# Layjins/Spider

Measured on AMD Instinct MI355X. Metric: multimodal responses/sec (text->text+image), higher is better.
Workload: dtype bf16

## Files before the change

include/spider_hip.h:

```cpp
#ifndef SPIDER_HIP_H
#define SPIDER_HIP_H
#define SPIDER_ABI_VERSION 4

#ifdef __cplusplus
extern "C" {
#endif

int spider_abi_version(void);
const char* spider_target_arch(void);
const char* spider_last_error(void);


int spider_embed_bf16(const void* table, const int* ids, void* out, int rows, int H, int V, void* stream);

int spider_rmsnorm_bf16(const void* x, const void* res, const void* w, void* y, void* res_out, int rows, int H,
                        float eps, void* stream);

int spider_gemv_bf16(const void* W, const void* x, void* out, const void* bias, const void* res, const void* norm_w,
                     float eps, int B, int N, int K, void* stream);

int spider_gemv_swiglu_bf16(const void* W_gate_up, const void* x, void* out, const void* norm_w, float eps, int B,
                            int I, int K, void* stream);

int spider_lm_head_nparts(int V);
// ... 18 lines not shown
                                         const int* ngram, const void* ban, void* ban_step, int V, int cap, int B, void* stream);

int spider_beam_partial_bf16(const void* logits, float* ws_ms, float* ws_val, int* ws_tok, int rows, int V, int C, int nslice,
                             void* stream);
int spider_beam_select_f32(const float* ws_ms, const float* ws_val, const int* ws_tok, float* run_scores, const int* eos_ids,
                           const int* n_eos, const int* n_hist, float* trace_score, int* trace_beam, int* trace_tok, int cap,
                           int* src_beam, int* next_ids, int B, int K, int V, int C, int nslice, void* stream);
int spider_kv_row_gather_bf16(void* k_cache, void* v_cache, void* k_tmp, void* v_tmp, const int* src_beam, const int* kv_beg,
                              const int* kv_end, int K, int R, int layers, int rows_alloc, int n_kv, int T, int d, void* stream);

int spider_sample_partial_bf16(const void* logits, const void* seen, const void* ban, const float* penalty, const int* min_new,
                               const int* eos_ids, const int* n_eos, const int* n_hist, const int* top_k, float* ws_val,
                               int* ws_tok, int rows, int V, int nslice, void* stream);
int spider_sample_select_f32(const float* ws_val, const int* ws_tok, const float* temperature, const float* top_p, const int* top_k,
                             const void* seed, const int* row0, const int* n_hist, int* next_ids, int* cand_tok, float* cand_p,
                             int* n_keep, float* u, int rows, int V, int nslice, void* stream);

int spider_rope_kv_append_bf16(const void* qkv, const int* pos, const int* slot, const float* cos_sin, void* q_out,
                               void* k_cache, void* v_cache, int B, int S, int n_q, int n_kv, int d, int T_max,
                               void* stream);
int spider_rope_kv_append_mrope_bf16(const void* qkv, const int* pos3, const int* slot, const float* cos_sin, void* q_out,
                                     void* k_cache, void* v_cache, int B, int S, int n_q, int n_kv, int d, int T_max,
                                     int sec_t, int sec_h, void* stream);

int spider_attn_decode_bf16(const void* q, const void* k_cache, const void* v_cache, const int* kv_beg,
                            const int* kv_end, void* out, void* ws_o, void* ws_ml, int B, int n_q, int n_kv, int d,
                            int T_max, float scale, int nsplit, void* stream);

int spider_attn_decode_fused_bf16(const void* qkv, const int* pos, const float* cos_sin, void* k_cache, void* v_cache,
                                  const int* kv_beg, const int* kv_end, void* out, void* ws_o, void* ws_ml,
                                  int* counters, int B, int n_q, int n_kv, int d, int T_max, float scale, int nsplit,
                                  void* stream);
int spider_set_attn_inline(int on);
int spider_set_gemv_sched(int sched);
int spider_set_ws_inlaunch(int on);

int spider_gemv_fm_bf16(const void* Wfm, const void* x, void* out, const void* bias, const void* res, int B, int N, int K,
                        int fold_rmsnorm, float eps, void* stream);
int spider_gemv_swiglu_fm_bf16(const void* Wfm_gate_up, const void* x, void* out, int B, int I, int K, int fold_rmsnorm, float eps,
                               void* stream);
int spider_lm_head_argmax_fm_bf16(const void* Wfm, const void* x, int* out_ids, void* logits, void* ws_val, void* ws_idx, int B,
                                  int V, int K, int fold_rmsnorm, float eps, void* stream);
int spider_lm_head_argmax_fm_proc_bf16(const void* Wfm, const void* x, int* out_ids, void* logits, void* ws_val, void* ws_idx,
                                       const void* seen, const void* ban, const float* penalty, const int* min_new,
                                       const int* eos_ids, const int* n_eos, const int* n_hist, int B, int V, int K,
                                       int fold_rmsnorm, float eps, void* stream);


int spider_gemm_bf16(const void* A, const void* W, void* C, void* C32, const void* bias, const void* res,
                     const void* rowbias, int rows_per_group, int M, int N, int K, int lda, int ldc, int act,
                     float out_scale, int w_tiled, const float* res32, float* c32d, void* ws, long ws_bytes, void* stream);

int spider_gemm_ln_bf16(const void* A, const void* Wf, void* C, const float* colsum, const float* colbias, const void* res,
                        int M, int N, int K, int ldc, int act, float eps, int w_tiled, void* ws, long ws_bytes, void* stream);

int spider_xattn_fused_bf16(const void* x, const void* mq_fm, const void* mo_fm, const float* colsum, const float* colbias,
                            const void* bias_o, void* out, int B2, int n_tok, int C, int heads, int n_keys, float eps,
                            const float* x32, float* out32, void* stream);

int spider_conv2d_nhwc_bf16(const void* x, const void* w, void* y, const void* bias, const void* res,
                            const void* rowbias, int B, int Hin, int Win, int Cin, int Cout, int ks, int stride,
                            int pad, int ups, float out_scale, int w_tiled, const float* res32, float* c32d, void* ws, long ws_bytes, void* stream);

int spider_conv_nhwc_ex_bf16(const void* x, const void* w, void* y, const void* bias, const void* res,
                             const void* rowbias, int B, int Hin, int Win, int Cin, int Cout, int kh, int kw, int stride,
                             int pad_h, int pad_w, int dil, int up_h, int up_w, int act, float act_param,
// ... 183 lines not shown
```

spider_amd/csrc/common.hpp:

```cpp
#pragma once
#include <hip/hip_runtime.h>
#include <stdint.h>

namespace spider {

typedef uint16_t bf16_t;

typedef __attribute__((ext_vector_type(4))) float f32x4;
typedef __attribute__((ext_vector_type(16))) float f32x16;
typedef __attribute__((ext_vector_type(8))) short bf16x8;
typedef __attribute__((ext_vector_type(4))) short bf16x4;

typedef __attribute__((ext_vector_type(4))) uint32_t u32x4;
typedef __attribute__((ext_vector_type(2))) uint32_t u32x2;

__device__ __forceinline__ float bf16_to_f32(bf16_t v) {
    return __uint_as_float(((uint32_t)v) << 16);
}
__device__ __forceinline__ float bf16lo_to_f32(uint32_t packed) {
    return __uint_as_float(packed << 16);
}
__device__ __forceinline__ float bf16hi_to_f32(uint32_t packed) {
    return __uint_as_float(packed & 0xffff0000u);
}
// ... 48 lines not shown
__device__ __forceinline__ float h16hi_to_f32(uint32_t packed) { return bf16hi_to_f32(packed); }
__device__ __forceinline__ h16_t f32_to_h16(float f) { return f32_to_bf16(f); }
__device__ __forceinline__ uint32_t pack_h16x2(float lo, float hi) { return pack_bf16x2(lo, hi); }
__device__ __forceinline__ float dot2_h16(uint32_t a, uint32_t b, float acc) {
    return __builtin_amdgcn_fdot2_f32_bf16(__builtin_bit_cast(hw_bf16x2, a), __builtin_bit_cast(hw_bf16x2, b), acc, false);
}
__device__ __forceinline__ f32x4 mfma_16x16x32_h16(h16x8 a, h16x8 b, f32x4 c) {
    return __builtin_amdgcn_mfma_f32_16x16x32_bf16(a, b, c, 0, 0, 0);
}
__device__ __forceinline__ f32x16 mfma_32x32x16_h16(h16x8 a, h16x8 b, f32x16 c) {
    return __builtin_amdgcn_mfma_f32_32x32x16_bf16(a, b, c, 0, 0, 0);
}
__device__ __forceinline__ f32x4 mfma_16x16x16_h16(h16x4 a, h16x4 b, f32x4 c) {
    return __builtin_amdgcn_mfma_f32_16x16x16bf16_1k(a, b, c, 0, 0, 0);
}
#endif
#define SPIDER_FN(name) SPIDER_CAT2(name, SPIDER_DT)

__device__ __forceinline__ float dot2_bf16(uint32_t a, uint32_t b, float acc) {
    return __builtin_amdgcn_fdot2_f32_bf16(__builtin_bit_cast(hw_bf16x2, a), __builtin_bit_cast(hw_bf16x2, b), acc, false);
}

__device__ __forceinline__ float wave_sum(float v) {
#pragma unroll
    for (int o = 32; o > 0; o >>= 1) v += __shfl_xor(v, o, 64);
    return v;
}
__device__ __forceinline__ float wave_max(float v) {
#pragma unroll
    for (int o = 32; o > 0; o >>= 1) v = fmaxf(v, __shfl_xor(v, o, 64));
    return v;
}

template <int NW>
__device__ __forceinline__ float block_sum(float v, float* red) {
    v = wave_sum(v);
    const int lane = threadIdx.x & 63, w = threadIdx.x >> 6;
    __syncthreads();
    if (lane == 0) red[w] = v;
    __syncthreads();
    float t = 0.f;
#pragma unroll
    for (int i = 0; i < NW; ++i) t += red[i];
    return t;
}

__device__ __forceinline__ float silu_f(float x) { return x * __builtin_amdgcn_rcpf(1.f + __expf(-x)); }
__device__ __forceinline__ float erf_fast(float x) {
    const float ax = fabsf(x);
    const float t = __builtin_amdgcn_rcpf(fmaf(0.3275911f, ax, 1.f));
    float p = fmaf(1.061405429f, t, -1.453152027f);
    p = fmaf(p, t, 1.421413741f);
    p = fmaf(p, t, -0.284496736f);
    p = fmaf(p, t, 0.254829592f);
    const float e = 1.f - p * t * __expf(-ax * ax);
    return copysignf(e, x);
}
__device__ __forceinline__ float gelu_erf_f(float x) { return 0.5f * x * (1.f + erf_fast(x * 0.70710678118654752f)); }
__device__ __forceinline__ float quick_gelu_f(float x) { return x * __builtin_amdgcn_rcpf(1.f + __expf(-1.702f * x)); }

__device__ __forceinline__ int xcd_remap(int bid, int nwg) {
    const int q = nwg >> 3, r = nwg & 7, xcd = bid & 7, idx = bid >> 3;
    const int base = (xcd < r) ? xcd * (q + 1) : r * (q + 1) + (xcd - r) * q;
    return base + idx;
}

}

template <typename F>
// ... 28 lines not shown
```

spider_amd/csrc/llm_decode.hip:

```cpp
#include "common.hpp"
#include "select.hpp"
#include <stdlib.h>

using namespace spider;

__global__ __launch_bounds__(256) void embed_kernel(const bf16_t* __restrict__ table, const int* __restrict__ ids,
                                                    bf16_t* __restrict__ out, int H, int V) {
    const int r = blockIdx.x;
    int id = ids[r];
    id = id < 0 ? 0 : (id >= V ? V - 1 : id);
    const u32x4* src = reinterpret_cast<const u32x4*>(table + (size_t)id * H);
    u32x4* dst = reinterpret_cast<u32x4*>(out + (size_t)r * H);
    for (int i = threadIdx.x; i < H / 8; i += 256) dst[i] = src[i];
}

__global__ __launch_bounds__(256) void rope_rows_kernel(bf16_t* __restrict__ x, const float* __restrict__ cs, long row_stride,
                                                        int rows, int heads, int d) {
    const int half = d >> 1, cpr = half >> 3;
    const long total = (long)rows * heads * cpr;
    for (long idx = (long)blockIdx.x * 256 + threadIdx.x; idx < total; idx += (long)gridDim.x * 256) {
        const int c = (int)(idx % cpr);
        const int h = (int)((idx / cpr) % heads);
        const long r = idx / ((long)cpr * heads);
        bf16_t* p = x + r * row_stride + (long)h * d + c * 8;
// ... 218 lines not shown
                u32x4 ov;
                ov.x = o[0]; ov.y = o[1]; ov.z = o[2]; ov.w = o[3];
                sv[min(i0 + c * NT, nv - 1)] = ov;
            }
        };
        auto hoist_w = [&]() {
#pragma unroll
            for (int u = 0; u < H; ++u) {
                const int k = lane * 8 + u * 512;
#pragma unroll
                for (int r = 0; r < NR; ++r)
                    w0[u][r] = __builtin_nontemporal_load(reinterpret_cast<const u32x4*>(wrow[r] + (unsigned)(k < K ? k : K - 8)));
            }
        };
        const u32x4* xv = reinterpret_cast<const u32x4*>(x);
        u32x4* sv = reinterpret_cast<u32x4*>(xs);
        if (!XLDS) {
            hoist_w();
        } else if (!norm_w) {
            issue_x(xv, t0);
            hoist_w();
            store_x(sv, t0);
            asm volatile("" ::: "memory");
            for (int b = 0; b < NB; ++b)
                for (int i0 = b ? 0 : CAP * NT; i0 < nv; i0 += CAP * NT) {
                    issue_x(xv + (size_t)b * nv, i0 + t0);
                    store_x(sv + (size_t)b * nv, i0 + t0);
                }
        } else if (nv <= CH * NT) {
            issue_xw(xv, t0);
            hoist_w();
            for (int b = 0; b < NB; ++b) {
                if (b) issue_xw(xv + (size_t)b * nv, t0);
                const float rs = rsqrtf(block_sum<NWB>(sumsq(0.f, t0, CH), red) / (float)K + eps);
                norm_store(sv + (size_t)b * nv, t0, rs);
            }
        } else {
            hoist_w();
            for (int b = 0; b < NB; ++b) {
                float ss = 0.f;
                for (int i0 = 0; i0 < nv; i0 += CAP * NT) {
                    issue_x(xv + (size_t)b * nv, i0 + t0);
                    ss = sumsq(ss, i0 + t0, CAP);
                }
                const float rs = rsqrtf(block_sum<NWB>(ss, red) / (float)K + eps);
                for (int i0 = 0; i0 < nv; i0 += CH * NT) {
                    issue_xw(xv + (size_t)b * nv, i0 + t0);
                    norm_store(sv + (size_t)b * nv, i0 + t0, rs);
                }
            }
        }
        if (XLDS) __syncthreads();
    }

    if (col0 >= N) return;
    float acc[NB][NR];
#pragma unroll
    for (int b = 0; b < NB; ++b)
#pragma unroll
        for (int r = 0; r < NR; ++r) acc[b][r] = 0.f;

    auto fma_w = [&](const u32x4 (&wq)[U][NR], int k0) {
#pragma unroll
        for (int u = 0; u < U; ++u) {
            const int k = k0 + u * 512;
            if (k < K) {
#pragma unroll
                for (int b = 0; b < NB; ++b) {
                    u32x4 xq = XLDS ? *reinterpret_cast<const u32x4*>(xs + (size_t)b * K + k)
                                    : *reinterpret_cast<const u32x4*>(x + (size_t)b * K + k);
                    const uint32_t xw[4] = {xq.x, xq.y, xq.z, xq.w};
#pragma unroll
                    for (int r = 0; r < NR; ++r) {
                        const uint32_t ww[4] = {wq[u][r].x, wq[u][r].y, wq[u][r].z, wq[u][r].w};
#pragma unroll
                        for (int j = 0; j < 4; ++j) acc[b][r] = dot2_bf16(ww[j], xw[j], acc[b][r]);
                    }
                }
// ... 65 lines not shown
            u32x4 wq[U][NR];
#pragma unroll
            for (int u = 0; u < U; ++u) {
                const int k = k0 + u * 512;
#pragma unroll
                for (int r = 0; r < NR; ++r)
                    wq[u][r] = __builtin_nontemporal_load(reinterpret_cast<const u32x4*>(wrow[r] + (unsigned)(k < K ? k : K - 8)));
            }
            fma_w(wq, k0);
        }
    } else {
        int kstart = lane * 8;
        if (hoist) {
            fma_w(w0, kstart);
            kstart += 512 * U;
        }
        for (int k0 = kstart; k0 < K; k0 += 512 * U) {
            u32x4 wq[U][NR];
#pragma unroll
            for (int u = 0; u < U; ++u) {
                const int k = k0 + u * 512;
                if (k < K) {
#pragma unroll
                    for (int r = 0; r < NR; ++r)
                        wq[u][r] = __builtin_nontemporal_load(reinterpret_cast<const u32x4*>(wrow[r] + k));
                }
            }
            fma_w(wq, k0);
        }
    }
#pragma unroll
    for (int b = 0; b < NB; ++b)
#pragma unroll
        for (int r = 0; r < NR; ++r) acc[b][r] = wave_sum(acc[b][r]);

    if (lane == 0) {
#pragma unroll
        for (int r = 0; r < R; ++r) {
            const int n = col0 + r;
            if (n < N) {
#pragma unroll
                for (int b = 0; b < NB; ++b) {
                    float v;
                    if (GATEUP) {
                        const float g = bf16_to_f32(f32_to_bf16(acc[b][r]));
                        const float u = bf16_to_f32(f32_to_bf16(acc[b][R + r]));
                        const float a = bf16_to_f32(f32_to_bf16(silu_f(g)));
                        v = a * u;
                    } else {
                        v = acc[b][r];
                        if (bias) v += bf16_to_f32(bias[n]);
                        if (res) v = bf16_to_f32(f32_to_bf16(v)) + bf16_to_f32(res[(size_t)b * N + n]);
                    }
                    out[(size_t)b * N + n] = f32_to_bf16(v);
                }
            }
        }
    }
}


template <int NB, int R, bool PROC = false>
__global__ __launch_bounds__(256) void lmhead_partial_kernel(const bf16_t* __restrict__ W, const bf16_t* __restrict__ x,
                                                             const bf16_t* __restrict__ norm_w, float eps,
                                                             float* __restrict__ pval, int* __restrict__ pidx,
                                                             bf16_t* __restrict__ logits, int V, int K, LmProc pr) {
    extern __shared__ __attribute__((aligned(16))) char smem[];
// ... 424 lines not shown
            ovv[u] = *reinterpret_cast<const float2*>(part_o + pi * D + lane * 2);
            if (!ok) mlv[u] = float2{-INFINITY, 0.f};
        }
#pragma unroll
        for (int u = 0; u < 16; ++u) {
            const float ms = mlv[u].x, ls = mlv[u].y;
            const float mn = fmaxf(m, ms);
            const float a = (m == -INFINITY) ? 0.f : __expf(m - mn);
            const float bsc = (ms == -INFINITY) ? 0.f : __expf(ms - mn);
            l = l * a + ls * bsc;
            o0 = o0 * a + ovv[u].x * bsc;
            o1 = o1 * a + ovv[u].y * bsc;
            m = mn;
        }
    }
    if (lane == 0) { sm_m[wave] = m; sm_l[wave] = l; }
    sm_o[wave][lane * 2] = o0;
    sm_o[wave][lane * 2 + 1] = o1;
    __syncthreads();
    if (threadIdx.x < D) {
        const int dd = threadIdx.x;
        float mm = fmaxf(fmaxf(sm_m[0], sm_m[1]), fmaxf(sm_m[2], sm_m[3]));
        float ll = 0.f, oo = 0.f;
#pragma unroll
        for (int w = 0; w < 4; ++w) {
            const float a = (sm_m[w] == -INFINITY) ? 0.f : __expf(sm_m[w] - mm);
            ll += sm_l[w] * a;
            oo += sm_o[w][dd] * a;
        }
        out[bh * D + dd] = f32_to_bf16(ll > 0.f ? oo / ll : 0.f);
    }
}

template <int D, int G, int NWV, int UR>
__global__ __launch_bounds__(NWV * 64) void attn_decode_fused_kernel(
    const bf16_t* __restrict__ qkv, const int* __restrict__ pos, const float* __restrict__ cs, bf16_t* __restrict__ kc,
    bf16_t* __restrict__ vc, const int* __restrict__ kv_beg, const int* __restrict__ kv_end, float* __restrict__ part_o,
    float* __restrict__ part_ml, int* __restrict__ cnt, bf16_t* __restrict__ out, int n_kv, int T_max, float scale,
    int nsplit, int inline_combine) {
    static_assert(D == 128, "decode attention is specialised for head_dim 128");
    constexpr int HALF = D / 2;
    const int split = blockIdx.x, hk = blockIdx.y, b = blockIdx.z;
    const int n_q = n_kv * G;
    const int lane = threadIdx.x & 63, wave = threadIdx.x >> 6;
    const int sub = lane >> 4;
    const int dl = (lane & 15) * 8;
    const bool hi_half = dl >= HALF;
    const int dp = hi_half ? dl - HALF : dl + HALF;
    const int beg = kv_beg ? kv_beg[b] : 0, end = kv_end[b];
    const int t_new = end - 1;
    const int len_old = max(t_new - beg, 0);
    const int per = (len_old + nsplit - 1) / nsplit;
    const int t0 = beg + split * per, t1 = min(t_new, t0 + per);

    const bf16_t* kbase = kc + ((size_t)b * n_kv + hk) * (size_t)T_max * D;
    const bf16_t* vbase = vc + ((size_t)b * n_kv + hk) * (size_t)T_max * D;
    constexpr int RSTEP = 4 * NWV;
    auto load_rows = [&](int tb_, u32x4 (&kr)[UR], u32x4 (&vr)[UR]) {
#pragma unroll
        for (int u = 0; u < UR; ++u) {
            const int t = min(tb_ + RSTEP * u, t1 - 1);
            kr[u] = *reinterpret_cast<const u32x4*>(kbase + (size_t)t * D + dl);
            vr[u] = *reinterpret_cast<const u32x4*>(vbase + (size_t)t * D + dl);
        }
    };
    const int tb0 = t0 + wave * 4 + sub;
    u32x4 kq[UR], vq[UR];
    if (tb0 < t1) load_rows(tb0, kq, vq);

    const bf16_t* row = qkv + (size_t)b * (n_q + 2 * n_kv) * D;
    const float* c = cs + (size_t)pos[b] * D;
    float cosv[8], sinv[8];
    {
        const int ci = hi_half ? dl - HALF : dl;
        const f32x4 c0 = *reinterpret_cast<const f32x4*>(c + ci), c1 = *reinterpret_cast<const f32x4*>(c + ci + 4);
        const f32x4 s0 = *reinterpret_cast<const f32x4*>(c + HALF + ci), s1 = *reinterpret_cast<const f32x4*>(c + HALF + ci + 4);
#pragma unroll
        for (int j = 0; j < 4; ++j) { cosv[j] = c0[j]; cosv[4 + j] = c1[j]; sinv[j] = s0[j]; sinv[4 + j] = s1[j]; }
    }
    auto rope8 = [&](const bf16_t* head, float (&o)[8]) {
        const u32x4 a = *reinterpret_cast<const u32x4*>(head + dl), pq = *reinterpret_cast<const u32x4*>(head + dp);
        const uint32_t aw[4] = {a.x, a.y, a.z, a.w}, pw[4] = {pq.x, pq.y, pq.z, pq.w};
#pragma unroll
        for (int j = 0; j < 8; ++j) {
            const float xv = (j & 1) ? bf16hi_to_f32(aw[j >> 1]) : bf16lo_to_f32(aw[j >> 1]);
            const float pv = (j & 1) ? bf16hi_to_f32(pw[j >> 1]) : bf16lo_to_f32(pw[j >> 1]);
            const float t1_ = bf16_to_f32(f32_to_bf16(xv * cosv[j]));
            const float t2_ = bf16_to_f32(f32_to_bf16((hi_half ? pv : -pv) * sinv[j]));
            o[j] = bf16_to_f32(f32_to_bf16(t1_ + t2_));
        }
    };

    float qf[G][8];
#pragma unroll
    for (int g = 0; g < G; ++g) {
        rope8(row + (size_t)(hk * G + g) * D, qf[g]);
#pragma unroll
        for (int j = 0; j < 8; ++j) qf[g][j] *= scale;
    }
    float m[G], l[G], o[G][8];
#pragma unroll
    for (int g = 0; g < G; ++g) {
        m[g] = -INFINITY;
        l[g] = 0.f;
#pragma unroll
        for (int j = 0; j < 8; ++j) o[g][j] = 0.f;
    }
    auto update = [&](const float (&kf)[8], const float (&vf)[8]) {
#pragma unroll
        for (int g = 0; g < G; ++g) {
            float sc = 0.f;
#pragma unroll
            for (int j = 0; j < 8; ++j) sc += qf[g][j] * kf[j];
            sc += __shfl_xor(sc, 1, 64);
            sc += __shfl_xor(sc, 2, 64);
            sc += __shfl_xor(sc, 4, 64);
            sc += __shfl_xor(sc, 8, 64);
            const float mn = fmaxf(m[g], sc);
            const float alpha = __expf(m[g] - mn);
            const float pr = __expf(sc - mn);
            l[g] = l[g] * alpha + pr;
#pragma unroll
            for (int j = 0; j < 8; ++j) o[g][j] = o[g][j] * alpha + pr * vf[j];
            m[g] = mn;
        }
    };

    constexpr int CHUNK = RSTEP * UR;
    for (int tb = tb0; tb < t1; tb += CHUNK) {
        const bool more = tb + CHUNK < t1;
#pragma unroll
        for (int u = 0; u < UR; ++u) {
            if (tb + RSTEP * u < t1) {
                const uint32_t kw[4] = {kq[u].x, kq[u].y, kq[u].z, kq[u].w}, vw[4] = {vq[u].x, vq[u].y, vq[u].z, vq[u].w};
                float kf[8], vf[8];
#pragma unroll
                for (int j = 0; j < 4; ++j) {
                    kf[2 * j] = bf16lo_to_f32(kw[j]); kf[2 * j + 1] = bf16hi_to_f32(kw[j]);
                    vf[2 * j] = bf16lo_to_f32(vw[j]); vf[2 * j + 1] = bf16hi_to_f32(vw[j]);
                }
                update(kf, vf);
            }
            if (more) {
                const int t = min(tb + CHUNK + RSTEP * u, t1 - 1);
                kq[u] = *reinterpret_cast<const u32x4*>(kbase + (size_t)t * D + dl);
                vq[u] = *reinterpret_cast<const u32x4*>(vbase + (size_t)t * D + dl);
            }
        }
    }
    if (split == nsplit - 1 && wave == 0 && sub == 0 && t_new >= beg) {
        float kf[8], vf[8];
        rope8(row + (size_t)(n_q + hk) * D, kf);
        const u32x4 vq = *reinterpret_cast<const u32x4*>(row + (size_t)(n_q + n_kv + hk) * D + dl);
        const uint32_t vw[4] = {vq.x, vq.y, vq.z, vq.w};
#pragma unroll
        for (int j = 0; j < 4; ++j) { vf[2 * j] = bf16lo_to_f32(vw[j]); vf[2 * j + 1] = bf16hi_to_f32(vw[j]); }
        update(kf, vf);
        u32x4 ko;
        ko.x = pack_bf16x2(kf[0], kf[1]); ko.y = pack_bf16x2(kf[2], kf[3]);
        ko.z = pack_bf16x2(kf[4], kf[5]); ko.w = pack_bf16x2(kf[6], kf[7]);
        *reinterpret_cast<u32x4*>(kc + (((size_t)b * n_kv + hk) * T_max + t_new) * D + dl) = ko;
        *reinterpret_cast<u32x4*>(vc + (((size_t)b * n_kv + hk) * T_max + t_new) * D + dl) = vq;
    }

    __shared__ float sm_m[NWV][G], sm_l[NWV][G];
    __shared__ float sm_o[NWV][G][D];
    __shared__ int sm_last;
#pragma unroll
    for (int g = 0; g < G; ++g) {
#pragma unroll
        for (int off = 16; off <= 32; off <<= 1) {
            const float m2 = __shfl_xor(m[g], off, 64);
            const float l2 = __shfl_xor(l[g], off, 64);
            const float mn = fmaxf(m[g], m2);
            const float a1 = (m[g] == -INFINITY) ? 0.f : __expf(m[g] - mn);
            const float a2 = (m2 == -INFINITY) ? 0.f : __expf(m2 - mn);
            l[g] = l[g] * a1 + l2 * a2;
#pragma unroll
            for (int j = 0; j < 8; ++j) {
                const float o2 = __shfl_xor(o[g][j], off, 64);
                o[g][j] = o[g][j] * a1 + o2 * a2;
            }
            m[g] = mn;
        }
        if (lane < 16) {
#pragma unroll
            for (int j = 0; j < 8; ++j) sm_o[wave][g][dl + j] = o[g][j];
            if (lane == 0) { sm_m[wave][g] = m[g]; sm_l[wave][g] = l[g]; }
        }
    }
    __syncthreads();
    if (nsplit > 1 && inline_combine) {
        for (int idx = threadIdx.x; idx < G * (D / 4); idx += NWV * 64) {
            const int g = idx / (D / 4), d4 = (idx % (D / 4)) * 4;
            float mm = -INFINITY;
#pragma unroll
            for (int w = 0; w < NWV; ++w) mm = fmaxf(mm, sm_m[w][g]);
            float ll = 0.f;
            f32x4 oo = {0.f, 0.f, 0.f, 0.f};
#pragma unroll
            for (int w = 0; w < NWV; ++w) {
                const float a = (sm_m[w][g] == -INFINITY) ? 0.f : __expf(sm_m[w][g] - mm);
                ll += sm_l[w][g] * a;
#pragma unroll
                for (int j = 0; j < 4; ++j) oo[j] += sm_o[w][g][d4 + j] * a;
            }
            const size_t pi = ((size_t)b * n_q + hk * G + g) * nsplit + split;
            float* po = part_o + pi * D + d4;
            asm volatile("global_store_dwordx4 %0, %1, off sc1" ::"v"(po), "v"(oo) : "memory");
            if (d4 == 0) {
                const float2 mlv = float2{mm, ll};
                float* pm = part_ml + pi * 2;
                asm volatile("global_store_dwordx2 %0, %1, off sc1" ::"v"(pm), "v"(mlv) : "memory");
            }
        }
        asm volatile("s_waitcnt vmcnt(0)" ::: "memory");
        __syncthreads();
        if (threadIdx.x == 0) {
            int ticket;
            if (inline_combine == 2) {
                ticket = __hip_atomic_fetch_add(cnt + (size_t)b * n_kv + hk, 1, __ATOMIC_RELAXED, __HIP_MEMORY_SCOPE_AGENT);
            } else {
// ... 18 lines not shown
                f32x4 ov[16];
                float2 mv[16];
#pragma unroll
                for (int u = 0; u < 16; ++u) {
                    const int sidx = min(s0 + u, nsplit - 1);
                    const uint32_t row = (uint32_t)(bh * nsplit + sidx);
                    ov[u] = __builtin_bit_cast(f32x4, __builtin_amdgcn_raw_buffer_load_b128(r_o, (row * D + d4) * 4u, 0, 16));
                    mv[u] = __builtin_bit_cast(float2, __builtin_amdgcn_raw_buffer_load_b64(r_ml, row * 8u, 0, 16));
                }
                float bm = mx;
#pragma unroll
                for (int u = 0; u < 16; ++u)
                    if (s0 + u < nsplit) bm = fmaxf(bm, mv[u].x);
                const float resc = (mx == -INFINITY) ? 0.f : __expf(mx - bm);
                lsum *= resc;
#pragma unroll
                for (int j = 0; j < 4; ++j) acc[j] *= resc;
                mx = bm;
#pragma unroll
                for (int u = 0; u < 16; ++u) {
                    const float w = (s0 + u < nsplit && mv[u].x != -INFINITY) ? __expf(mv[u].x - mx) : 0.f;
                    lsum += mv[u].y * w;
#pragma unroll
                    for (int j = 0; j < 4; ++j) acc[j] += ov[u][j] * w;
                }
            }
            const float inv = lsum > 0.f ? 1.f / lsum : 0.f;
            u32x2 o2;
            o2.x = pack_bf16x2(acc[0] * inv, acc[1] * inv);
            o2.y = pack_bf16x2(acc[2] * inv, acc[3] * inv);
            *reinterpret_cast<u32x2*>(out + bh * D + d4) = o2;
        }
        if (threadIdx.x == 0) __hip_atomic_store(cnt + (size_t)b * n_kv + hk, 0, __ATOMIC_RELAXED, __HIP_MEMORY_SCOPE_AGENT);
        return;
    }
    for (int idx = threadIdx.x; idx < G * D; idx += NWV * 64) {
        const int g = idx / D, dd = idx % D;
        float mm = -INFINITY;
#pragma unroll
        for (int w = 0; w < NWV; ++w) mm = fmaxf(mm, sm_m[w][g]);
        float ll = 0.f, oo = 0.f;
#pragma unroll
        for (int w = 0; w < NWV; ++w) {
            const float a = (sm_m[w][g] == -INFINITY) ? 0.f : __expf(sm_m[w][g] - mm);
            ll += sm_l[w][g] * a;
            oo += sm_o[w][g][dd] * a;
        }
        const int hq = hk * G + g;
        if (nsplit == 1) {
            out[((size_t)b * n_q + hq) * D + dd] = f32_to_bf16(ll > 0.f ? oo / ll : 0.f);
        } else {
            const size_t pi = ((size_t)b * n_q + hq) * nsplit + split;
            part_o[pi * D + dd] = oo;
            if (dd == 0) { part_ml[pi * 2] = mm; part_ml[pi * 2 + 1] = ll; }
        }
    }
}

template <bool GATEUP, int NW>
__global__ __launch_bounds__(NW * 64) void skinny_gemm_kernel(const bf16_t* __restrict__ W, const bf16_t* __restrict__ x,
                                                          bf16_t* __restrict__ out, const bf16_t* __restrict__ bias,
                                                          const bf16_t* __restrict__ res, int B, int N, int K) {
    constexpr int TN = GATEUP ? 2 : 1;
    __shared__ float part[NW][TN][64][4];
    const int lane = threadIdx.x & 63, wave = threadIdx.x >> 6;
    const int r16 = lane & 15, g = lane >> 4;
// ... 292 lines not shown
    else GEMV_PICK(4);
#undef GEMV_PICK
    SPIDER_LAUNCH_OK();
    return 0;
}

template <bool GU>
static int gemv_batch(const void* W, const void* x, void* out, const void* bias, const void* res, const void* norm_w,
                      float eps, int B, int N, int K, void* stream) {
    static const int mfma_min_b = [] { const char* e = getenv("SPIDER_GEMV_MFMA_MIN_B"); return e ? atoi(e) : 5; }();
    if (B >= mfma_min_b && B <= 16 && K % 64 == 0 && norm_w == nullptr) {
        skinny_gemm_kernel<GU, 8><<<(N + 15) / 16, 512, 0, (hipStream_t)stream>>>((const bf16_t*)W, (const bf16_t*)x, (bf16_t*)out,
                                                                                  (const bf16_t*)bias, (const bf16_t*)res, B, N, K);
        SPIDER_LAUNCH_OK();
        return 0;
    }
    switch (B) {
        case 1: return gemv_dispatch<1, GU>(W, x, out, bias, res, norm_w, eps, N, K, stream);
        case 2: return gemv_dispatch<2, GU>(W, x, out, bias, res, norm_w, eps, N, K, stream);
        case 3: return gemv_dispatch<3, GU>(W, x, out, bias, res, norm_w, eps, N, K, stream);
        case 4: return gemv_dispatch<4, GU>(W, x, out, bias, res, norm_w, eps, N, K, stream);
        case 5: return gemv_dispatch<5, GU>(W, x, out, bias, res, norm_w, eps, N, K, stream);
        case 6: return gemv_dispatch<6, GU>(W, x, out, bias, res, norm_w, eps, N, K, stream);
        case 7: return gemv_dispatch<7, GU>(W, x, out, bias, res, norm_w, eps, N, K, stream);
        case 8: return gemv_dispatch<8, GU>(W, x, out, bias, res, norm_w, eps, N, K, stream);
        default: spider_set_error("gemv: batch must be 1..8 (1..16 when K % 64 == 0 and norm_w == NULL; use spider_gemm_bf16 beyond that)"); return -1;
    }
}


#define SPIDER_ATTN_INLINE_DEFAULT 0
static int g_attn_inline = -1;

extern "C" {

int spider_set_gemv_sched(int sched) {
    const int prev = gemv_sched();
    g_gemv_sched = sched != 0;
    return prev;
}

int spider_set_attn_inline(int on) {
    const int prev = g_attn_inline;
    g_attn_inline = on < 0 ? 0 : (on > 2 ? 2 : on);
    return prev;
}

int spider_embed_bf16(const void* table, const int* ids, void* out, int rows, int H, int V, void* stream) {
    SPIDER_CHECK(rows > 0 && H > 0 && H % 8 == 0 && V > 0, "embed: bad shape (H must be a multiple of 8)");
    embed_kernel<<<rows, 256, 0, (hipStream_t)stream>>>((const bf16_t*)table, ids, (bf16_t*)out, H, V);
    SPIDER_LAUNCH_OK();
    return 0;
}

int spider_rope_rows_bf16(void* x, const float* cos_sin, long row_stride, int rows, int heads, int d, void* stream) {
    SPIDER_CHECK(rows > 0 && heads > 0 && d > 0 && d % 16 == 0, "rope_rows: head_dim must be a multiple of 16");
    SPIDER_CHECK(row_stride % 8 == 0 && row_stride >= (long)heads * d, "rope_rows: row stride must be >= heads*d and keep 16-byte alignment");
    const long total = (long)rows * heads * (d / 16);
    long g = (total + 255) / 256;
    if (g > 8192) g = 8192;
    rope_rows_kernel<<<(int)g, 256, 0, (hipStream_t)stream>>>((bf16_t*)x, cos_sin, row_stride, rows, heads, d);
    SPIDER_LAUNCH_OK();
    return 0;
}

int spider_rmsnorm_bf16(const void* x, const void* res, const void* w, void* y, void* res_out, int rows, int H,
                        float eps, void* stream) {
// ... 243 lines not shown
int spider_attn_decode_bf16(const void* q, const void* k_cache, const void* v_cache, const int* kv_beg,
                            const int* kv_end, void* out, void* ws_o, void* ws_ml, int B, int n_q, int n_kv, int d,
                            int T_max, float scale, int nsplit, void* stream) {
    SPIDER_CHECK(d == 128, "attn_decode: head_dim must be 128");
    SPIDER_CHECK(B > 0 && n_kv > 0 && n_q % n_kv == 0 && nsplit >= 1 && T_max > 0, "attn_decode: bad shape");
    SPIDER_CHECK(nsplit == 1 || (ws_o && ws_ml), "attn_decode: workspace required for nsplit > 1");
    const int G = n_q / n_kv;
    dim3 grid(nsplit, n_kv, B);
    switch (G) {
        case 1: ATTN_DEC_LAUNCH(1); break;
        case 2: ATTN_DEC_LAUNCH(2); break;
        case 3: ATTN_DEC_LAUNCH(3); break;
        case 4: ATTN_DEC_LAUNCH(4); break;
        case 5: ATTN_DEC_LAUNCH(5); break;
        case 6: ATTN_DEC_LAUNCH(6); break;
        case 7: ATTN_DEC_LAUNCH(7); break;
        case 8: ATTN_DEC_LAUNCH(8); break;
        default: spider_set_error("attn_decode: GQA group size must be 1 ... 8"); return -1;
    }
    SPIDER_LAUNCH_OK();
    if (nsplit > 1) {
        attn_combine_kernel<128><<<B * n_q, 256, 0, (hipStream_t)stream>>>((const float*)ws_o, (const float*)ws_ml,
                                                                          (bf16_t*)out, nsplit);
        SPIDER_LAUNCH_OK();
    }
    return 0;
}

#define ATTN_FUSED_ARGS                                                                                         \
    (const bf16_t*)qkv, pos, cos_sin, (bf16_t*)k_cache, (bf16_t*)v_cache, kv_beg, kv_end, (float*)ws_o, (float*)ws_ml, counters, \
        (bf16_t*)out, n_kv, T_max, scale, nsplit, inline_combine
#define ATTN_FUSED_LAUNCH(G_)                                                                                   \
    do {                                                                                                        \
        if (wide) attn_decode_fused_kernel<128, G_, 8, 8><<<grid, 512, 0, (hipStream_t)stream>>>(ATTN_FUSED_ARGS); \
        else attn_decode_fused_kernel<128, G_, 4, 4><<<grid, 256, 0, (hipStream_t)stream>>>(ATTN_FUSED_ARGS);   \
    } while (0)

int spider_attn_decode_fused_bf16(const void* qkv, const int* pos, const float* cos_sin, void* k_cache, void* v_cache,
                                  const int* kv_beg, const int* kv_end, void* out, void* ws_o, void* ws_ml,
                                  int* counters, int B, int n_q, int n_kv, int d, int T_max, float scale, int nsplit,
                                  void* stream) {
    SPIDER_CHECK(d == 128, "attn_decode_fused: head_dim must be 128");
    SPIDER_CHECK(B > 0 && n_kv > 0 && n_q % n_kv == 0 && nsplit >= 1 && T_max > 0, "attn_decode_fused: bad shape");
    SPIDER_CHECK(nsplit == 1 || (ws_o && ws_ml && counters), "attn_decode_fused: workspace + counters required for nsplit > 1");
    const int G = n_q / n_kv;
    dim3 grid(nsplit, n_kv, B);
    if (g_attn_inline < 0) { const char* e = getenv("SPIDER_ATTN_INLINE"); g_attn_inline = e ? (atoi(e) < 0 ? 0 : (atoi(e) > 2 ? 2 : atoi(e))) : SPIDER_ATTN_INLINE_DEFAULT; }
    const int inline_combine = g_attn_inline;
    static const int wide_env = [] { const char* e = getenv("SPIDER_ATTN_WIDE"); return e ? atoi(e) : -1; }();
    const bool wide = wide_env >= 0 ? wide_env != 0 : (T_max / nsplit >= 96);
    switch (G) {
        case 1: ATTN_FUSED_LAUNCH(1); break;
        case 2: ATTN_FUSED_LAUNCH(2); break;
        case 3: ATTN_FUSED_LAUNCH(3); break;
        case 4: ATTN_FUSED_LAUNCH(4); break;
        case 5: ATTN_FUSED_LAUNCH(5); break;
        case 6: ATTN_FUSED_LAUNCH(6); break;
        case 7: ATTN_FUSED_LAUNCH(7); break;
        case 8: ATTN_FUSED_LAUNCH(8); break;
        default: spider_set_error("attn_decode_fused: GQA group size must be 1 ... 8"); return -1;
    }
    SPIDER_LAUNCH_OK();
    if (nsplit > 1 && !inline_combine) {
        attn_combine_kernel<128><<<B * n_q, 256, 0, (hipStream_t)stream>>>((const float*)ws_o, (const float*)ws_ml,
                                                                          (bf16_t*)out, nsplit);
        SPIDER_LAUNCH_OK();
    }
    return 0;
}

}
```

spider_amd/lib.py:

```python
from __future__ import annotations

import ctypes as C
import os
import threading

import torch

_HERE = os.path.dirname(os.path.abspath(__file__))
LIB_PATH = os.path.join(_HERE, "libspider_hip.so")

_lib = None
_lock = threading.Lock()

_vp, _i, _f, _l = C.c_void_p, C.c_int, C.c_float, C.c_long

SIGNATURES = {
    "spider_abi_version": (_i, []),
    "spider_target_arch": (C.c_char_p, []),
    "spider_last_error": (C.c_char_p, []),
    "spider_embed_bf16": (_i, [_vp, _vp, _vp, _i, _i, _i, _vp]),
    "spider_rmsnorm_bf16": (_i, [_vp, _vp, _vp, _vp, _vp, _i, _i, _f, _vp]),
    "spider_gemv_bf16": (_i, [_vp, _vp, _vp, _vp, _vp, _vp, _f, _i, _i, _i, _vp]),
    "spider_gemv_swiglu_bf16": (_i, [_vp, _vp, _vp, _vp, _f, _i, _i, _i, _vp]),
    "spider_lm_head_nparts": (_i, [_i]),
    "spider_decode_advance_i32": (_i, [_vp] * 7 + [_i, _i, _vp]),
    "spider_lm_head_argmax_bf16": (_i, [_vp, _vp, _vp, _f, _vp, _vp, _vp, _vp, _i, _i, _i, _vp]),
    "spider_lm_head_argmax_proc_bf16": (_i, [_vp, _vp, _vp, _f] + [_vp] * 11 + [_i, _i, _i, _vp]),
    "spider_decode_advance_seen_i32": (_i, [_vp] * 8 + [_i, _i, _i, _vp]),
    "spider_token_bitmap_set_i32": (_i, [_vp, _vp, _i, _i, _i, _vp]),
    "spider_ngram_ban_i32": (_i, [_vp, _vp, _i, _vp, _vp, _i, _vp, _vp, _vp, _i, _i, _vp]),
    "spider_decode_advance_seen_ngram_i32": (_i, [_vp] * 10 + [_i] + [_vp] * 3 + [_i] * 3 + [_vp]),
    "spider_beam_partial_bf16": (_i, [_vp] * 4 + [_i] * 4 + [_vp]),
    "spider_beam_select_f32": (_i, [_vp] * 10 + [_i, _vp, _vp] + [_i] * 5 + [_vp]),
    "spider_kv_row_gather_bf16": (_i, [_vp] * 7 + [_i] * 7 + [_vp]),
    "spider_sample_partial_bf16": (_i, [_vp] * 11 + [_i] * 3 + [_vp]),
    "spider_sample_select_f32": (_i, [_vp] * 13 + [_i] * 3 + [_vp]),
    "spider_gemv_fm_bf16": (_i, [_vp, _vp, _vp, _vp, _vp, _i, _i, _i, _i, _f, _vp]),
    "spider_gemv_swiglu_fm_bf16": (_i, [_vp, _vp, _vp, _i, _i, _i, _i, _f, _vp]),
    "spider_lm_head_argmax_fm_bf16": (_i, [_vp, _vp, _vp, _vp, _vp, _vp, _i, _i, _i, _i, _f, _vp]),
    "spider_lm_head_argmax_fm_proc_bf16": (_i, [_vp] * 13 + [_i, _i, _i, _i, _f, _vp]),
    "spider_rope_kv_append_bf16": (_i, [_vp, _vp, _vp, _vp, _vp, _vp, _vp, _i, _i, _i, _i, _i, _i, _vp]),
    "spider_rope_kv_append_mrope_bf16": (_i, [_vp, _vp, _vp, _vp, _vp, _vp, _vp, _i, _i, _i, _i, _i, _i, _i, _i, _vp]),
    "spider_attn_decode_bf16": (_i, [_vp, _vp, _vp, _vp, _vp, _vp, _vp, _vp, _i, _i, _i, _i, _i, _f, _i, _vp]),
    "spider_attn_decode_fused_bf16": (_i, [_vp] * 11 + [_i, _i, _i, _i, _i, _f, _i, _vp]),
    "spider_set_attn_inline": (_i, [_i]),
    "spider_set_gemv_sched": (_i, [_i]),
    "spider_set_ws_inlaunch": (_i, [_i]),
    "spider_gemm_bf16": (_i, [_vp, _vp, _vp, _vp, _vp, _vp, _vp, _i, _i, _i, _i, _i, _i, _i, _f, _i, _vp, _vp, _vp, _l, _vp]),
    "spider_gemm_ln_bf16": (_i, [_vp, _vp, _vp, _vp, _vp, _vp, _i, _i, _i, _i, _i, _f, _i, _vp, _l, _vp]),
    "spider_xattn_fused_bf16": (_i, [_vp, _vp, _vp, _vp, _vp, _vp, _vp, _i, _i, _i, _i, _i, _f, _vp, _vp, _vp]),
    "spider_conv2d_nhwc_bf16": (_i, [_vp, _vp, _vp, _vp, _vp, _vp, _i, _i, _i, _i, _i, _i, _i, _i, _i, _f, _i, _vp, _vp, _vp, _l, _vp]),
    "spider_conv_nhwc_ex_bf16": (_i, [_vp] * 6 + [_i] * 14 + [_f, _f, _i, _vp, _vp, _vp, _l, _vp]),
    "spider_attn_bf16": (_i, [_vp, _vp, _vp, _vp] + [_l] * 12 + [_i] * 6 + [_f, _i, _i, _vp, _vp, _i, _i, _vp]),
    "spider_story_key_lists_i32": (_i, [_vp, _i, _i, _i, _i, _i, _i, _vp, _vp, _vp]),
    "spider_attn_keylist_bf16": (_i, [_vp, _vp, _vp, _vp] + [_l] * 12 + [_i] * 6 + [_f, _vp, _i, _vp, _i, _vp]),
    "spider_attn_varlen_bf16": (_i, [_vp, _vp, _vp, _vp, _l, _l, _l, _l, _i, _i, _i, _i, _f, _vp, _i, _vp]),
    "spider_rope_rows_bf16": (_i, [_vp, _vp, _l, _i, _i, _i, _vp]),
    "spider_groupnorm_nchunk": (_i, [_i]),
    "spider_groupnorm_nhwc_bf16": (_i, [_vp, _vp, _vp, _vp, _vp, _i, _i, _i, _i, _f, _i, _vp]),
    "spider_groupnorm_cat_nhwc_bf16": (_i, [_vp] * 7 + [_i, _i, _i, _i, _i, _f, _i, _vp]),
    "spider_conv_nhwc_gn_bf16": (_i, [_vp] * 6 + [_i] * 14 + [_f, _f, _i, _vp, _vp, _vp, _l, _vp] + [_vp, _i, _vp]),
    "spider_groupnorm_stats_nhwc_bf16": (_i, [_vp, _vp, _i, _i, _i, _i, _i, _vp]),
    "spider_groupnorm_apply_nhwc_bf16": (_i, [_vp, _vp, _i, _vp, _vp, _vp, _i, _i, _i, _i, _f, _i, _vp]),
    "spider_gemm_gn_in_bf16": (_i, [_vp, _vp, _vp, _vp, _i, _i, _i, _i, _i, _vp, _i, _vp, _vp, _i, _f, _i, _vp, _vp]),
    "spider_layernorm_bf16": (_i, [_vp, _vp, _vp, _vp, _i, _i, _f, _vp]),
    "spider_geglu_bf16": (_i, [_vp, _vp, _i, _i, _vp]),
    "spider_swiglu_bf16": (_i, [_vp, _vp, _i, _i, _vp]),
    "spider_concat_channels_bf16": (_i, [_vp, _vp, _vp, _l, _i, _i, _vp]),
    "spider_act_bf16": (_i, [_vp, _vp, _l, _i, _vp]),
    "spider_add_bf16": (_i, [_vp, _vp, _vp, _l, _vp]),
    "spider_act_ex_bf16": (_i, [_vp, _vp, _l, _i, _f, _vp]),
    "spider_add_scaled_bf16": (_i, [_vp, _vp, _vp, _l, _f, _vp]),
    "spider_axpby_bf16": (_i, [_vp, _vp, _vp, _l, _f, _f, _vp]),
    "spider_mean_tokens_bf16": (_i, [_vp, _vp, _i, _i, _i, _vp]),
    "spider_moe_combine_bf16": (_i, [_vp, _i, _vp, _i, _vp, _i, _l, _vp]),
    "spider_col2im1d_f32_bf16": (_i, [_vp, _vp, _vp, _i, _i, _i, _i, _i, _i, _vp]),
    "spider_l2_normalize_rows_bf16": (_i, [_vp, _vp, _i, _i, _f, _vp]),
    "spider_conv2d_small_cin_bf16": (_i, [_vp, _vp, _vp, _vp, _i, _i, _i, _i, _i, _i, _vp]),
# ... 68 lines not shown
```

Measured before the change: 2.030.

## Use DPP/permlane cross-lane reductions in decode attention, gemv, and rmsnorm

Adds DPP and permlane-swap based lane-xor helpers and uses them instead of ds_bpermute shuffles for wave reductions in the fused decode attention kernel, the scheduled gemv path, and the folded rmsnorm block sums. The attention kernel also computes RoPE'd q once per head in shared memory instead of every wave recomputing all G heads. It merges wave partials with permlane swaps and vectorises the cross-wave combine. The goal is to cut LDS-routed shuffle latency and redundant q work in the memory-bound decode step. The cost is an extra syncthreads and shared buffer, plus a reliance on gfx950 permlane builtins.

```diff
diff --git a/include/spider_hip.h b/include/spider_hip.h
--- a/include/spider_hip.h
+++ b/include/spider_hip.h
@@ -74,6 +74,7 @@
                                   int* counters, int B, int n_q, int n_kv, int d, int T_max, float scale, int nsplit,
                                   void* stream);
 int spider_set_attn_inline(int on);
+int spider_set_attn_xlane(int on);
 int spider_set_gemv_sched(int sched);
 int spider_set_ws_inlaunch(int on);
 
diff --git a/spider_amd/csrc/common.hpp b/spider_amd/csrc/common.hpp
--- a/spider_amd/csrc/common.hpp
+++ b/spider_amd/csrc/common.hpp
@@ -104,9 +104,72 @@
     return v;
 }
 
-template <int NW>
+template <int M>
+__device__ __forceinline__ uint32_t lane_xor(uint32_t u) {
+    static_assert(M == 1 || M == 2 || M == 4 || M == 8 || M == 16 || M == 32, "lane_xor: M must be a power of two below 64");
+    if constexpr (M == 1) {
+        return (uint32_t)__builtin_amdgcn_update_dpp(0, (int)u, 0xB1, 0xf, 0xf, true);
+    } else if constexpr (M == 2) {
+        return (uint32_t)__builtin_amdgcn_update_dpp(0, (int)u, 0x4E, 0xf, 0xf, true);
+    } else if constexpr (M == 4) {
+        const int t = __builtin_amdgcn_update_dpp(0, (int)u, 0x141, 0xf, 0xf, true);
+        return (uint32_t)__builtin_amdgcn_update_dpp(0, t, 0x1B, 0xf, 0xf, true);
+    } else if constexpr (M == 8) {
+        return (uint32_t)__builtin_amdgcn_update_dpp(0, (int)u, 0x128, 0xf, 0xf, true);
+    } else if constexpr (M == 16) {
+        const auto r = __builtin_amdgcn_permlane16_swap(u, u, false, false);
+        return (threadIdx.x & 16) ? r[0] : r[1];
+    } else {
+        const auto r = __builtin_amdgcn_permlane32_swap(u, u, false, false);
+        return (threadIdx.x & 32) ? r[0] : r[1];
+    }
+}
+template <int M>
+__device__ __forceinline__ float lane_xor(float v) { return __uint_as_float(lane_xor<M>(__float_as_uint(v))); }
+template <int M>
+__device__ __forceinline__ int lane_xor(int v) { return (int)lane_xor<M>((uint32_t)v); }
+template <int M>
+__device__ __forceinline__ float lane_xor_lo(float v) {
+    static_assert(M == 16 || M == 32, "lane_xor_lo: M must be 16 or 32");
+    const uint32_t u = __float_as_uint(v);
+    if constexpr (M == 16) return __uint_as_float(__builtin_amdgcn_permlane16_swap(u, u, false, false)[1]);
+    else return __uint_as_float(__builtin_amdgcn_permlane32_swap(u, u, false, false)[1]);
+}
+template <int M>
+__device__ __forceinline__ float xor_add(float v) {
+    if constexpr (M == 16) {
+        const auto r = __builtin_amdgcn_permlane16_swap(__float_as_uint(v), __float_as_uint(v), false, false);
+        return __uint_as_float(r[0]) + __uint_as_float(r[1]);
+    } else if constexpr (M == 32) {
+        const auto r = __builtin_amdgcn_permlane32_swap(__float_as_uint(v), __float_as_uint(v), false, false);
+        return __uint_as_float(r[0]) + __uint_as_float(r[1]);
+    } else {
+        return v + lane_xor<M>(v);
+    }
+}
+template <int M>
+__device__ __forceinline__ float xor_max(float v) {
+    if constexpr (M == 16) {
+        const auto r = __builtin_amdgcn_permlane16_swap(__float_as_uint(v), __float_as_uint(v), false, false);
+        return fmaxf(__uint_as_float(r[0]), __uint_as_float(r[1]));
+    } else if constexpr (M == 32) {
+        const auto r = __builtin_amdgcn_permlane32_swap(__float_as_uint(v), __float_as_uint(v), false, false);
+        return fmaxf(__uint_as_float(r[0]), __uint_as_float(r[1]));
+    } else {
+        return fmaxf(v, lane_xor<M>(v));
+    }
+}
+__device__ __forceinline__ float wave_sum_valu(float v) {
+    return xor_add<1>(xor_add<2>(xor_add<4>(xor_add<8>(xor_add<16>(xor_add<32>(v))))));
+}
+__device__ __forceinline__ float wave_max_valu(float v) {
+    return xor_max<1>(xor_max<2>(xor_max<4>(xor_max<8>(xor_max<16>(xor_max<32>(v))))));
+}
+__device__ __forceinline__ float row16_sum_valu(float v) { return xor_add<8>(xor_add<4>(xor_add<2>(xor_add<1>(v)))); }
+
+template <int NW, bool VALU = false>
 __device__ __forceinline__ float block_sum(float v, float* red) {
-    v = wave_sum(v);
+    v = VALU ? wave_sum_valu(v) : wave_sum(v);
     const int lane = threadIdx.x & 63, w = threadIdx.x >> 6;
     __syncthreads();
     if (lane == 0) red[w] = v;
diff --git a/spider_amd/csrc/llm_decode.hip b/spider_amd/csrc/llm_decode.hip
--- a/spider_amd/csrc/llm_decode.hip
+++ b/spider_amd/csrc/llm_decode.hip
@@ -274,7 +274,7 @@
             hoist_w();
             for (int b = 0; b < NB; ++b) {
                 if (b) issue_xw(xv + (size_t)b * nv, t0);
-                const float rs = rsqrtf(block_sum<NWB>(sumsq(0.f, t0, CH), red) / (float)K + eps);
+                const float rs = rsqrtf(block_sum<NWB, true>(sumsq(0.f, t0, CH), red) / (float)K + eps);
                 norm_store(sv + (size_t)b * nv, t0, rs);
             }
         } else {
@@ -285,7 +285,7 @@
                     issue_x(xv + (size_t)b * nv, i0 + t0);
                     ss = sumsq(ss, i0 + t0, CAP);
                 }
-                const float rs = rsqrtf(block_sum<NWB>(ss, red) / (float)K + eps);
+                const float rs = rsqrtf(block_sum<NWB, true>(ss, red) / (float)K + eps);
                 for (int i0 = 0; i0 < nv; i0 += CH * NT) {
                     issue_xw(xv + (size_t)b * nv, i0 + t0);
                     norm_store(sv + (size_t)b * nv, i0 + t0, rs);
@@ -417,7 +417,7 @@
 #pragma unroll
     for (int b = 0; b < NB; ++b)
 #pragma unroll
-        for (int r = 0; r < NR; ++r) acc[b][r] = wave_sum(acc[b][r]);
+        for (int r = 0; r < NR; ++r) acc[b][r] = SCHED ? wave_sum_valu(acc[b][r]) : wave_sum(acc[b][r]);
 
     if (lane == 0) {
 #pragma unroll
@@ -908,7 +908,7 @@
     }
 }
 
-template <int D, int G, int NWV, int UR>
+template <int D, int G, int NWV, int UR, bool XL = false>
 __global__ __launch_bounds__(NWV * 64) void attn_decode_fused_kernel(
     const bf16_t* __restrict__ qkv, const int* __restrict__ pos, const float* __restrict__ cs, bf16_t* __restrict__ kc,
     bf16_t* __restrict__ vc, const int* __restrict__ kv_beg, const int* __restrict__ kv_end, float* __restrict__ part_o,
@@ -945,9 +945,11 @@
     if (tb0 < t1) load_rows(tb0, kq, vq);
 
     const bf16_t* row = qkv + (size_t)b * (n_q + 2 * n_kv) * D;
-    const float* c = cs + (size_t)pos[b] * D;
-    float cosv[8], sinv[8];
-    {
+    const int gi = wave * 4 + sub;
+    const bool rot = !XL || gi < G;
+    float cosv[8] = {0.f, 0.f, 0.f, 0.f, 0.f, 0.f, 0.f, 0.f}, sinv[8] = {0.f, 0.f, 0.f, 0.f, 0.f, 0.f, 0.f, 0.f};
+    if (rot) {
+        const float* c = cs + (size_t)pos[b] * D;
         const int ci = hi_half ? dl - HALF : dl;
         const f32x4 c0 = *reinterpret_cast<const f32x4*>(c + ci), c1 = *reinterpret_cast<const f32x4*>(c + ci + 4);
         const f32x4 s0 = *reinterpret_cast<const f32x4*>(c + HALF + ci), s1 = *reinterpret_cast<const f32x4*>(c + HALF + ci + 4);
@@ -968,11 +970,31 @@
     };
 
     float qf[G][8];
-#pragma unroll
-    for (int g = 0; g < G; ++g) {
-        rope8(row + (size_t)(hk * G + g) * D, qf[g]);
-#pragma unroll
-        for (int j = 0; j < 8; ++j) qf[g][j] *= scale;
+    if constexpr (XL) {
+        __shared__ __attribute__((aligned(16))) float sm_q[G][D];
+        if (gi < G) {
+            float qr[8];
+            rope8(row + (size_t)(hk * G + gi) * D, qr);
+            f32x4 q0, q1;
+#pragma unroll
+            for (int j = 0; j < 4; ++j) { q0[j] = qr[j] * scale; q1[j] = qr[4 + j] * scale; }
+            *reinterpret_cast<f32x4*>(&sm_q[gi][dl]) = q0;
+            *reinterpret_cast<f32x4*>(&sm_q[gi][dl + 4]) = q1;
+        }
+        __syncthreads();
+#pragma unroll
+        for (int g = 0; g < G; ++g) {
+            const f32x4 q0 = *reinterpret_cast<const f32x4*>(&sm_q[g][dl]), q1 = *reinterpret_cast<const f32x4*>(&sm_q[g][dl + 4]);
+#pragma unroll
+            for (int j = 0; j < 4; ++j) { qf[g][j] = q0[j]; qf[g][4 + j] = q1[j]; }
+        }
+    } else {
+#pragma unroll
+        for (int g = 0; g < G; ++g) {
+            rope8(row + (size_t)(hk * G + g) * D, qf[g]);
+#pragma unroll
+            for (int j = 0; j < 8; ++j) qf[g][j] *= scale;
+        }
     }
     float m[G], l[G], o[G][8];
 #pragma unroll
@@ -988,16 +1010,21 @@
             float sc = 0.f;
 #pragma unroll
             for (int j = 0; j < 8; ++j) sc += qf[g][j] * kf[j];
-            sc += __shfl_xor(sc, 1, 64);
-            sc += __shfl_xor(sc, 2, 64);
-            sc += __shfl_xor(sc, 4, 64);
-            sc += __shfl_xor(sc, 8, 64);
+            if constexpr (XL) {
+                sc = row16_sum_valu(sc);
+            } else {
+                sc += __shfl_xor(sc, 1, 64);
+                sc += __shfl_xor(sc, 2, 64);
+                sc += __shfl_xor(sc, 4, 64);
+                sc += __shfl_xor(sc, 8, 64);
+            }
             const float mn = fmaxf(m[g], sc);
             const float alpha = __expf(m[g] - mn);
             const float pr = __expf(sc - mn);
             l[g] = l[g] * alpha + pr;
 #pragma unroll
-            for (int j = 0; j < 8; ++j) o[g][j] = o[g][j] * alpha + pr * vf[j];
+            for (int j = 0; j < 8; ++j)
+                o[g][j] = j < 2 ? __builtin_fmaf(o[g][j], alpha, pr * vf[j]) : __builtin_fmaf(pr, vf[j], o[g][j] * alpha);
             m[g] = mn;
         }
     };
@@ -1040,8 +1067,39 @@
     }
 
     __shared__ float sm_m[NWV][G], sm_l[NWV][G];
-    __shared__ float sm_o[NWV][G][D];
+    __shared__ __attribute__((aligned(16))) float sm_o[NWV][G][D];
     __shared__ int sm_last;
+    if constexpr (XL) {
+        auto merge = [&](int g, auto xl) {
+            const float m2 = xl(m[g]), l2 = xl(l[g]);
+            const float mn = fmaxf(m[g], m2);
+            const float a1 = (m[g] == -INFINITY) ? 0.f : __expf(m[g] - mn);
+            const float a2 = (m2 == -INFINITY) ? 0.f : __expf(m2 - mn);
+            l[g] = __builtin_fmaf(l[g], a1, l2 * a2);
+#pragma unroll
+            for (int j = 0; j < 8; ++j) {
+                const float o2 = xl(o[g][j]);
+                o[g][j] = __builtin_fmaf(o[g][j], a1, o2 * a2);
+            }
+            m[g] = mn;
+        };
+#pragma unroll
+        for (int g = 0; g < G; ++g) {
+            merge(g, [](float v) { return lane_xor_lo<16>(v); });
+            merge(g, [](float v) { return lane_xor_lo<32>(v); });
+        }
+        if (lane < 16) {
+#pragma unroll
+            for (int g = 0; g < G; ++g) {
+                f32x4 o0, o1;
+#pragma unroll
+                for (int j = 0; j < 4; ++j) { o0[j] = o[g][j]; o1[j] = o[g][4 + j]; }
+                *reinterpret_cast<f32x4*>(&sm_o[wave][g][dl]) = o0;
+                *reinterpret_cast<f32x4*>(&sm_o[wave][g][dl + 4]) = o1;
+                if (lane == 0) { sm_m[wave][g] = m[g]; sm_l[wave][g] = l[g]; }
+            }
+        }
+    } else {
 #pragma unroll
     for (int g = 0; g < G; ++g) {
 #pragma unroll
@@ -1051,11 +1109,11 @@
             const float mn = fmaxf(m[g], m2);
             const float a1 = (m[g] == -INFINITY) ? 0.f : __expf(m[g] - mn);
             const float a2 = (m2 == -INFINITY) ? 0.f : __expf(m2 - mn);
-            l[g] = l[g] * a1 + l2 * a2;
+            l[g] = __builtin_fmaf(l[g], a1, l2 * a2);
 #pragma unroll
             for (int j = 0; j < 8; ++j) {
                 const float o2 = __shfl_xor(o[g][j], off, 64);
-                o[g][j] = o[g][j] * a1 + o2 * a2;
+                o[g][j] = __builtin_fmaf(o[g][j], a1, o2 * a2);
             }
             m[g] = mn;
         }
@@ -1064,6 +1122,7 @@
             for (int j = 0; j < 8; ++j) sm_o[wave][g][dl + j] = o[g][j];
             if (lane == 0) { sm_m[wave][g] = m[g]; sm_l[wave][g] = l[g]; }
         }
+    }
     }
     __syncthreads();
     if (nsplit > 1 && inline_combine) {
@@ -1148,6 +1207,36 @@
             *reinterpret_cast<u32x2*>(out + bh * D + d4) = o2;
         }
         if (threadIdx.x == 0) __hip_atomic_store(cnt + (size_t)b * n_kv + hk, 0, __ATOMIC_RELAXED, __HIP_MEMORY_SCOPE_AGENT);
+        return;
+    }
+    if constexpr (XL) {
+        for (int idx = threadIdx.x; idx < G * (D / 4); idx += NWV * 64) {
+            const int g = idx / (D / 4), d4 = (idx % (D / 4)) * 4;
+            float mm = -INFINITY;
+#pragma unroll
+            for (int w = 0; w < NWV; ++w) mm = fmaxf(mm, sm_m[w][g]);
+            float ll = 0.f;
+            f32x4 oo = {0.f, 0.f, 0.f, 0.f};
+#pragma unroll
+            for (int w = 0; w < NWV; ++w) {
+                const float a = (sm_m[w][g] == -INFINITY) ? 0.f : __expf(sm_m[w][g] - mm);
+                ll += sm_l[w][g] * a;
+                const f32x4 ov = *reinterpret_cast<const f32x4*>(&sm_o[w][g][d4]);
+#pragma unroll
+                for (int j = 0; j < 4; ++j) oo[j] += ov[j] * a;
+            }
+            const int hq = hk * G + g;
+            if (nsplit == 1) {
+                u32x2 o2;
+                o2.x = pack_bf16x2(ll > 0.f ? oo[0] / ll : 0.f, ll > 0.f ? oo[1] / ll : 0.f);
+                o2.y = pack_bf16x2(ll > 0.f ? oo[2] / ll : 0.f, ll > 0.f ? oo[3] / ll : 0.f);
+                *reinterpret_cast<u32x2*>(out + ((size_t)b * n_q + hq) * D + d4) = o2;
+            } else {
+                const size_t pi = ((size_t)b * n_q + hq) * nsplit + split;
+                *reinterpret_cast<f32x4*>(part_o + pi * D + d4) = oo;
+                if (d4 == 0) *reinterpret_cast<float2*>(part_ml + pi * 2) = float2{mm, ll};
+            }
+        }
         return;
     }
     for (int idx = threadIdx.x; idx < G * D; idx += NWV * 64) {
@@ -1506,7 +1595,19 @@
 #define SPIDER_ATTN_INLINE_DEFAULT 0
 static int g_attn_inline = -1;
 
+static int g_attn_xlane = -1;
+static int attn_xlane() {
+    if (g_attn_xlane < 0) { const char* e = getenv("SPIDER_ATTN_XLANE"); g_attn_xlane = e ? (atoi(e) != 0) : 1; }
+    return g_attn_xlane;
+}
+
 extern "C" {
+
+int spider_set_attn_xlane(int on) {
+    const int prev = attn_xlane();
+    g_attn_xlane = on != 0;
+    return prev;
+}
 
 int spider_set_gemv_sched(int sched) {
     const int prev = gemv_sched();
@@ -1816,7 +1917,9 @@
         (bf16_t*)out, n_kv, T_max, scale, nsplit, inline_combine
 #define ATTN_FUSED_LAUNCH(G_)                                                                                   \
     do {                                                                                                        \
-        if (wide) attn_decode_fused_kernel<128, G_, 8, 8><<<grid, 512, 0, (hipStream_t)stream>>>(ATTN_FUSED_ARGS); \
+        if (wide && xlane) attn_decode_fused_kernel<128, G_, 8, 8, true><<<grid, 512, 0, (hipStream_t)stream>>>(ATTN_FUSED_ARGS); \
+        else if (wide) attn_decode_fused_kernel<128, G_, 8, 8><<<grid, 512, 0, (hipStream_t)stream>>>(ATTN_FUSED_ARGS); \
+        else if (xlane) attn_decode_fused_kernel<128, G_, 4, 4, true><<<grid, 256, 0, (hipStream_t)stream>>>(ATTN_FUSED_ARGS); \
         else attn_decode_fused_kernel<128, G_, 4, 4><<<grid, 256, 0, (hipStream_t)stream>>>(ATTN_FUSED_ARGS);   \
     } while (0)
 
@@ -1831,6 +1934,7 @@
     dim3 grid(nsplit, n_kv, B);
     if (g_attn_inline < 0) { const char* e = getenv("SPIDER_ATTN_INLINE"); g_attn_inline = e ? (atoi(e) < 0 ? 0 : (atoi(e) > 2 ? 2 : atoi(e))) : SPIDER_ATTN_INLINE_DEFAULT; }
     const int inline_combine = g_attn_inline;
+    const bool xlane = attn_xlane() != 0;
     static const int wide_env = [] { const char* e = getenv("SPIDER_ATTN_WIDE"); return e ? atoi(e) : -1; }();
     const bool wide = wide_env >= 0 ? wide_env != 0 : (T_max / nsplit >= 96);
     switch (G) {
diff --git a/spider_amd/lib.py b/spider_amd/lib.py
--- a/spider_amd/lib.py
+++ b/spider_amd/lib.py
@@ -44,6 +44,7 @@
     "spider_attn_decode_bf16": (_i, [_vp, _vp, _vp, _vp, _vp, _vp, _vp, _vp, _i, _i, _i, _i, _i, _f, _i, _vp]),
     "spider_attn_decode_fused_bf16": (_i, [_vp] * 11 + [_i, _i, _i, _i, _i, _f, _i, _vp]),
     "spider_set_attn_inline": (_i, [_i]),
+    "spider_set_attn_xlane": (_i, [_i]),
     "spider_set_gemv_sched": (_i, [_i]),
     "spider_set_ws_inlaunch": (_i, [_i]),
     "spider_gemm_bf16": (_i, [_vp, _vp, _vp, _vp, _vp, _vp, _vp, _i, _i, _i, _i, _i, _i, _i, _f, _i, _vp, _vp, _vp, _l, _vp]),
```

Result: faster. 2.071, median of 6 (+2.0%).
